# ml-unito/PartitionedLS.jl

Hardware: NVIDIA B200
Metric: opt_fit_orthant_nnls_solves_per_sec (higher is better)
Workload: dtype f64

## Files before the change

### partitionedls.jl_b200/csrc/nnls5.cu

```cuda
#include "common.cuh"

namespace pls {
namespace {

constexpr int H5_BYTES_ = 192;
constexpr int SG_FREE5 = 2;
constexpr unsigned char ST_INO = 1;
constexpr unsigned char ST_PAS = 2;
constexpr unsigned char ST_BLK = 4;
constexpr unsigned char ST_FAST = 8;
#define SYNC5() __syncthreads()

__device__ __forceinline__ void dmma5(double &d0, double &d1, double a, double b) {
  asm("mma.sync.aligned.m8n8k4.row.col.f64.f64.f64.f64 {%0,%1}, {%2}, {%3}, {%0,%1};\n"
      : "+d"(d0), "+d"(d1) : "d"(a), "d"(b));
}
__device__ __forceinline__ double rcp5(double x) {
  double r;
  asm("rcp.approx.ftz.f64 %0, %1;" : "=d"(r) : "d"(x));
  double e = fma(-x, r, 1.0);
  r = fma(r, e, r);
  e = fma(-x, r, 1.0);
  return fma(r, e, r);
}
__device__ __forceinline__ double wmax5(double v) {
#pragma unroll
  for (int o = 16; o; o >>= 1) v = fmax(v, __shfl_xor_sync(0xffffffffu, v, o));
  return v;
}
__host__ __device__ constexpr int t2_doubles(int nr) { return ((nr / 8) * (nr / 8 + 1) / 2) * 64; }
__device__ __forceinline__ int t2_idx(int i, int j) {
  const int ti = i >> 3, tj = j >> 3;
  return ((((ti * (ti + 1)) >> 1) + tj) << 6) + ((i & 7) << 3) + (j & 7);
}
__device__ __forceinline__ double t2_get(const double *T2, int i, int j) { return i >= j ? T2[t2_idx(i, j)] : T2[t2_idx(j, i)]; }
__device__ __forceinline__ void t2_set(double *T2, int i, int j, double v) {
  const int a = i > j ? i : j, b = i > j ? j : i;
  const int x = t2_idx(a, b);
  T2[x] = v;
  if ((a >> 3) == (b >> 3)) T2[x - ((a & 7) << 3) - (b & 7) + ((b & 7) << 3) + (a & 7)] = v;
}
__device__ __forceinline__ int pan5(int row, int col) { return (row << 3) + (col ^ ((row & 2) << 1)); }

struct Sh5 {
  double *T2;
  double *v;
  double *Pp, *Wp;
  double *yv;
  double *D;
  double *gd;
  double *red;
  int4 *binfo;
  int *ctl;
  short *slot;
  short *rvar;
  short *lst;
  short *lstE;
  short *lstB;
  unsigned short *tmap;
  signed char *sg;
  unsigned char *st;
  unsigned char *grp;
  unsigned char *mk;
};
enum { C_NS = 0, C_OK, C_CNT, C_N, C_NJ, C_NP, C_NLV, C_FLAG };

__host__ __device__ inline size_t sh5_bytes(int NR, int ld1) {
  const int ntl = (NR / 8) * (NR / 8 + 1) / 2;
  return H5_BYTES_ + sizeof(double) * ((size_t)t2_doubles(NR) + ld1 + 16 * (size_t)NR + NR + 64 + 8 + 32 + 16) + sizeof(int) * 16 +
         sizeof(short) * (2 * (size_t)ld1 + 2 * (size_t)NR + 8 + ((ntl + 3) & ~3)) + 3 * (size_t)ld1 + NR + 16 + 16;
}

__device__ __forceinline__ Sh5 make_sh5(int NR, int ld1) {
  extern __shared__ __align__(16) unsigned char smem_raw5[];
  const int ntl = (NR / 8) * (NR / 8 + 1) / 2;
  Sh5 s;
  double *dp = reinterpret_cast<double *>(smem_raw5 + H5_BYTES_);
  s.T2 = dp; dp += t2_doubles(NR);
  s.Pp = dp; dp += 8 * NR;
  s.Wp = dp; dp += 8 * NR;
  s.yv = dp; dp += NR;
  s.D = dp; dp += 64;
  s.gd = dp; dp += 8;
  s.red = dp; dp += 32;
  s.binfo = reinterpret_cast<int4 *>(dp); dp += 16;
  int *ip = reinterpret_cast<int *>(dp);
  s.ctl = ip; ip += 16;
  short *sp = reinterpret_cast<short *>(ip);
  s.rvar = sp; sp += NR;
  s.lstE = sp; sp += NR;
  s.lstB = sp; sp += 8;
  s.tmap = reinterpret_cast<unsigned short *>(sp); sp += (ntl + 3) & ~3;
  s.mk = reinterpret_cast<unsigned char *>(sp);
  dp = reinterpret_cast<double *>(smem_raw5 + ((static_cast<int>(s.mk - smem_raw5) + NR + 15) & ~15));
  s.v = dp; dp += ld1;
  sp = reinterpret_cast<short *>(dp);
  s.slot = sp; sp += ld1;
  s.lst = sp; sp += ld1;
  signed char *cp = reinterpret_cast<signed char *>(sp);
  s.sg = cp; cp += ld1;
  s.st = reinterpret_cast<unsigned char *>(cp); cp += ld1;
  s.grp = reinterpret_cast<unsigned char *>(cp);
  return s;
}

struct H5 {
  double *T1;
  const double *T1r;
  double *Pg;
  const double *G;
  const unsigned long long *gmask;
  int ld1, nr, Mp, ldg;
  int cold_fused;
  int gen;
  int pad0, pad1;
  unsigned long long cnt[10];
  double yy, cmax;
  double max_viol;
};
enum { H_SWEEP = 0, H_STREAM, H_SUMS, H_SUMP2, H_ITER, H_BLK, H_REBUILD, H_FOLD, H_DRIFT, H_NOCONV };
constexpr int H5_BYTES = H5_BYTES_;
static_assert(sizeof(H5) <= H5_BYTES, "header size");
__device__ __forceinline__ H5 &hdr5() {
  extern __shared__ __align__(16) unsigned char smem_raw5[];
  return *reinterpret_cast<H5 *>(smem_raw5);
}

template <int T>
__device__ __forceinline__ double bmax5(const Sh5 &s, double v) {
  constexpr int NW = T / 32;
  v = wmax5(v);
  if ((threadIdx.x & 31) == 0) s.red[threadIdx.x >> 5] = v;
  SYNC5();
  double r = s.red[0];
#pragma unroll
  for (int i = 1; i < NW; ++i) r = fmax(r, s.red[i]);
  SYNC5();
  return r;
}

template <int T>
__device__ __forceinline__ void set_block5(const Sh5 &s, int nb, int slot) {
  const int tid = threadIdx.x;
  const H5 &h = hdr5();
  const int g = h.gen;
  if (g == 1) {
    #pragma unroll 1
    for (int k = tid; k < h.nr; k += T) s.mk[k] = 0;
    SYNC5();
  }
  if (tid < nb) {
    const int tc = slot >> 3, c7 = slot & 7;
    s.lstB[tid] = (short)slot;
    s.binfo[tid] = make_int4(slot, (tc << 6) + c7, (((tc * (tc + 1)) >> 1) << 6) + (c7 << 3), 0);
    s.mk[slot] = (unsigned char)g;
  }
}

template <int T, int NR>
__device__ __noinline__ int t2_block(int n, int nb, int nlv, bool test, bool flip) {
  H5 &h = hdr5();
  const int gen = h.gen;
  const Sh5 s = make_sh5(NR, h.ld1);
  constexpr int NW = T / 32;
  const int tid = threadIdx.x, lane = tid & 31, wid = tid >> 5;
  const int fr = lane >> 2, fk = lane & 3;
  const int ntr = (n + 7) >> 3;
  const short *B = s.lstB;
  if (tid >= 32 || T == 32) {
    constexpr int TG = T == 32 ? 32 : T - 32;
#pragma unroll 1
    for (int row = T == 32 ? tid : tid - 32; row < ntr * 8; row += TG) {
      const int tr = row >> 3, r7 = row & 7;
      const int rbase = (((tr * (tr + 1)) >> 1) << 6) + (r7 << 3), rowt = (tr << 6) + r7;
      const int sw = (row & 2) << 1, pb = row << 3;
#pragma unroll 1
      for (int q = 0; q < 8; ++q) {
        double val = 0.0;
        if (row < n && q < nb) { const int4 bi = s.binfo[q]; val = s.T2[row >= bi.x ? rbase + bi.y : bi.z + rowt]; }
        s.Pp[pb + (q ^ sw)] = val;
      }
    }
  }
  if (tid < 32) {
    if (lane < 8) {
      s.gd[lane] = (test && lane >= nlv && lane < nb) ? 1e-13 * __ldg(h.G + (size_t)h.ldg * s.rvar[B[lane]] + s.rvar[B[lane]]) : 0.0;
    }
    const int i = lane >> 2, j0 = (lane & 3) << 1;
    double e0 = (i < nb && j0 < nb) ? t2_get(s.T2, B[i], B[j0]) : (i == j0 ? 1.0 : 0.0);
    double e1 = (i < nb && j0 + 1 < nb) ? t2_get(s.T2, B[i], B[j0 + 1]) : (i == j0 + 1 ? 1.0 : 0.0);
    int bad = nb;
#pragma unroll 1
    for (int k = 0; k < nb; ++k) {
      __syncwarp();
      s.D[i * 8 + j0] = e0; s.D[i * 8 + j0 + 1] = e1;
      __syncwarp();
      const double pk0 = s.D[k * 8 + j0], pk1 = s.D[k * 8 + j0 + 1], cik = s.D[i * 8 + k], pkk = s.D[k * 8 + k];
      const bool good = k < nlv ? pkk < 0.0 : (test ? pkk > s.gd[k] : pkk > 0.0);
      if (!good && bad == nb) bad = k;
      const double d = rcp5(pkk), fct = cik * d;
      const bool rowk = i == k;
      double n0 = rowk ? pk0 * d : fma(-fct, pk0, e0);
      double n1 = rowk ? pk1 * d : fma(-fct, pk1, e1);
      if (j0 == k) n0 = rowk ? d : -fct;
      if (j0 + 1 == k) n1 = rowk ? d : -fct;
      e0 = n0; e1 = n1;
    }
    __syncwarp();
    s.D[i * 8 + j0] = e0; s.D[i * 8 + j0 + 1] = e1;
    if (lane == 0) s.ctl[C_OK] = bad == nb ? nb : (bad < nlv ? -1 : bad);
  }
  SYNC5();
  const int res = s.ctl[C_OK];
  if (tid == 0) h.gen = gen == 255 ? 1 : gen + 1;
  if (res != nb) { SYNC5(); return res; }
  #pragma unroll 1
  for (int ti = wid; ti < ntr; ti += NW) {
    double c0 = 0.0, c1 = 0.0;
// ... 23 lines not shown
    }
  }
  SYNC5();
#pragma unroll 1
  for (int row = tid; row < n; row += T) {
    if (s.mk[row] == (unsigned char)gen) continue;
    const int tr = row >> 3, r7 = row & 7;
    const int rbase = (((tr * (tr + 1)) >> 1) << 6) + (r7 << 3), rowt = (tr << 6) + r7;
    const int sw = (row & 2) << 1, pb = row << 3;
#pragma unroll 1
    for (int q = 0; q < nb; ++q) {
      const int4 bi = s.binfo[q];
      const int tc = bi.x >> 3;
      const double w0 = s.Wp[pb + (q ^ sw)];
      const double val = q < nlv ? -w0 : w0;
      if (tr >= tc) s.T2[rbase + bi.y] = val;
      if (tr <= tc) s.T2[bi.z + rowt] = val;
    }
  }
#pragma unroll 1
  for (int e = tid; e < 64; e += T) {
    const int i = e >> 3, j = e & 7;
    if (i < nb && j <= i) { const double val = s.D[i * 8 + j]; t2_set(s.T2, B[i], B[j], ((i < nlv) == (j < nlv)) ? -val : val); }
  }
  if (flip && tid < nb) s.st[s.rvar[B[tid]]] ^= ST_PAS;
  SYNC5();
  if (tid == 0) { h.cnt[H_SWEEP] += nb; h.cnt[H_SUMP2] += ((unsigned long long)(n * n) * nb) >> 2; }
  return nb;
}

template <int T, int NR>
__device__ __noinline__ bool t2_rebuild(int n) {
  const H5 &h = hdr5();
  const Sh5 s = make_sh5(NR, h.ld1);
  constexpr int NW = T / 32;
  const int tid = threadIdx.x, lane = tid & 31, wid = tid >> 5;
  #pragma unroll 1
  for (int i = wid; i < n; i += NW) {
    const double *row = h.T1r + (size_t)h.ld1 * s.rvar[i];
    #pragma unroll 1
    for (int j = lane; j <= i; j += 32) t2_set(s.T2, i, j, __ldcg(row + s.rvar[j]));
  }
  if (tid < 32) {
    int cnt = 0, nlv = 0;
    #pragma unroll 1
    for (int pass = 0; pass < 2; ++pass) {
      #pragma unroll 1
      for (int k0 = 1; k0 < n; k0 += 32) {
        const int k = k0 + lane;
        bool take = false;
        if (k < n) { const unsigned char f = s.st[s.rvar[k]]; const bool pas = f & ST_PAS, ino = f & ST_INO; take = pas != ino && (pass == 0 ? !pas : pas); }
        const unsigned bal = __ballot_sync(0xffffffffu, take);
        if (take) s.lst[cnt + __popc(bal & ((1u << lane) - 1))] = (short)k;
        cnt += __popc(bal);
      }
      if (pass == 0) nlv = cnt;
    }
    if (lane == 0) { s.ctl[C_CNT] = cnt; s.ctl[C_NLV] = nlv; }
  }
  SYNC5();
  const int cnt = s.ctl[C_CNT], nlv = s.ctl[C_NLV];
  #pragma unroll 1
  for (int q0 = 0; q0 < cnt; q0 += 8) {
    const int nb = min(8, cnt - q0);
    set_block5<T>(s, nb, tid < nb ? s.lst[q0 + tid] : 0);
    SYNC5();
    if (t2_block<T, NR>(n, nb, max(0, min(nb, nlv - q0)), false, false) != nb) return false;
  }
  return true;
}

template <int NR>
__device__ __noinline__ int window_reset() {
  const H5 &h = hdr5();
  const Sh5 s = make_sh5(NR, h.ld1);
  const int tid = threadIdx.x;
  const int Mp = h.Mp;
  if (tid < 32) {
    const int lane = tid;
    if (lane == 0) s.rvar[0] = (short)Mp;
    int base = 1;
    #pragma unroll 1
    for (int m0 = 0; m0 < Mp; m0 += 32) {
      const int m = m0 + lane;
      bool keep = false;
      if (m < Mp) {
        const unsigned char f = s.st[m];
        keep = (f & ST_FAST) || (((f & ST_PAS) != 0) != ((f & ST_INO) != 0));
      }
      const unsigned bal = __ballot_sync(0xffffffffu, keep);
      if (m < Mp) {
        if (keep) { const int k = base + __popc(bal & ((1u << lane) - 1)); s.rvar[k] = (short)m; s.slot[m] = (short)k; }
        else s.slot[m] = -1;
      }
      base += __popc(bal);
    }
    if (lane == 0) s.ctl[C_N] = base;
  }
  SYNC5();
  return s.ctl[C_N];
}

template <int T, int NR>
__device__ __noinline__ int t2_compact(int n) {
  const H5 &h = hdr5();
  const Sh5 s = make_sh5(NR, h.ld1);
  const int tid = threadIdx.x;
  double *scr = h.Pg + 8 * (size_t)h.ld1;
  short *old = s.lst;
  if (tid < 32) {
    const int lane = tid;
    if (lane == 0) old[0] = 0;
    int base = 1;
    #pragma unroll 1
    for (int k0 = 1; k0 < n; k0 += 32) {
      const int k = k0 + lane;
      bool keep = false; int m = 0;
      if (k < n) {
        m = s.rvar[k];
        const unsigned char f = s.st[m];
        keep = (f & ST_FAST) || (((f & ST_PAS) != 0) != ((f & ST_INO) != 0));
      }
      const unsigned bal = __ballot_sync(0xffffffffu, keep);
      const int kn = base + __popc(bal & ((1u << lane) - 1));
      __syncwarp();
      if (k < n) {
        if (keep) { old[kn] = (short)k; s.rvar[kn] = (short)m; s.slot[m] = (short)kn; }
        else s.slot[m] = -1;
      }
      __syncwarp();
      base += __popc(bal);
    }
    if (lane == 0) s.ctl[C_N] = base;
  }
  SYNC5();
  const int nn = s.ctl[C_N];
  if (nn == n) return n;
  #pragma unroll 1
  for (int idx = tid; idx < nn * nn; idx += T) {
    const int a = idx / nn, b = idx - a * nn;
    if (b <= a) __stcg(scr + idx, t2_get(s.T2, old[a], old[b]));
  }
  __threadfence_block();
  SYNC5();
  #pragma unroll 1
  for (int idx = tid; idx < nn * nn; idx += T) {
    const int a = idx / nn, b = idx - a * nn;
    if (b <= a) t2_set(s.T2, a, b, __ldcg(scr + idx));
  }
  SYNC5();
  return nn;
}

template <int T, int NQ, int NR>
__device__ __noinline__ void stream5(int n) {
  const H5 &h = hdr5();
  const Sh5 s = make_sh5(NR, h.ld1);
  const int tid = threadIdx.x;
  const int ld2 = h.ld1 >> 1;
  constexpr int UB = 8;
  constexpr int NG = T >= 512 ? 2 : 1, TG = T / NG, NQE = NQ * NG, UBG = UB * NG;
  const int grp = NG == 1 ? 0 : tid / TG, lt = NG == 1 ? tid : tid - grp * TG;
  int ns = 0;
  {
    constexpr int NW = T / 32;
    const int lane = tid & 31, wid = tid >> 5;
    int *ri = reinterpret_cast<int *>(s.red);
    #pragma unroll 1
    for (int k0 = 1; k0 < n; k0 += T) {
      const int k = k0 + tid;
      bool tg = false, pas = false; int m = 0;
      if (k < n) { m = s.rvar[k]; const unsigned char f = s.st[m]; pas = f & ST_PAS; tg = pas != ((f & ST_INO) != 0); }
      const unsigned bal = __ballot_sync(0xffffffffu, tg);
      if (k0 > 1) SYNC5();
      if (lane == 0) ri[wid] = __popc(bal);
      SYNC5();
      int off = ns;
#pragma unroll
      for (int w2 = 0; w2 < NW; ++w2) { const int c = ri[w2]; if (w2 < wid) off += c; ns += c; }
      if (tg) { const int p = off + __popc(bal & ((1u << lane) - 1)); s.lst[p] = (short)m; const double t = s.T2[t2_idx(k, 0)]; s.yv[p] = pas ? t : -t; }
    }
    const int nsp = (ns + UBG - 1) / UBG * UBG;
    #pragma unroll 1
    for (int p = ns + tid; p < nsp; p += T) { s.lst[p] = (short)h.Mp; s.yv[p] = 0.0; }
    if (tid == 0) { s.ctl[C_NS] = ns; s.ctl[C_FLAG] = 0; }
  }
  SYNC5();
  const int nsp = (ns + UBG - 1) / UBG * UBG;
  double2 acc[NQE];
  const double2 *T1v = reinterpret_cast<const double2 *>(h.T1r);
  {
    const double2 *r = T1v + (size_t)ld2 * h.Mp;
#pragma unroll
    for (int q = 0; q < NQE; ++q) acc[q] = (grp == 0 && lt + TG * q < ld2) ? __ldcg(r + lt + TG * q) : make_double2(0.0, 0.0);
  }
  #pragma unroll 1
  for (int p = 0; p < nsp; p += UBG) {
    double2 g[UB][NQE];
#pragma unroll
    for (int u = 0; u < UB; ++u) {
      const double2 *r = T1v + (size_t)ld2 * s.lst[p + u * NG + grp];
#pragma unroll
      for (int q = 0; q < NQE; ++q) g[u][q] = (lt + TG * q < ld2) ? __ldcg(r + lt + TG * q) : make_double2(0.0, 0.0);
    }
#pragma unroll
    for (int u = 0; u < UB; ++u) {
      const double y = s.yv[p + u * NG + grp];
#pragma unroll
      for (int q = 0; q < NQE; ++q) { acc[q].x = fma(-y, g[u][q].x, acc[q].x); acc[q].y = fma(-y, g[u][q].y, acc[q].y); }
    }
  }
  if (NG > 1) {
    double2 *scr = reinterpret_cast<double2 *>(s.Wp);
    if (grp == 1) {
#pragma unroll
      for (int q = 0; q < NQE; ++q) if (lt + TG * q < ld2) scr[lt + TG * q] = acc[q];
    }
    SYNC5();
    if (grp == 0) {
#pragma unroll
      for (int q = 0; q < NQE; ++q) if (lt + TG * q < ld2) { const double2 o = scr[lt + TG * q]; acc[q].x += o.x; acc[q].y += o.y; }
    }
  }
  if (grp == 0) {
#pragma unroll
    for (int q = 0; q < NQE; ++q)
      if (lt + TG * q < ld2) reinterpret_cast<double2 *>(s.v)[lt + TG * q] = acc[q];
  }
  SYNC5();
  if (tid == 0) { hdr5().cnt[H_STREAM]++; hdr5().cnt[H_SUMS] += ns; }
}

template <int T, int NR>
__device__ __noinline__ int join_block5(int n, const short *Jl, int nj) {
  const H5 &h = hdr5();
  const Sh5 s = make_sh5(NR, h.ld1);
  constexpr int NW = T / 32, TPW = (NR / 8 + NW - 1) / NW;
  const int tid = threadIdx.x, lane = tid & 31, wid = tid >> 5;
  const int fr = lane >> 2, fk = lane & 3;
  const size_t ld1 = h.ld1;
  const double *T1r = h.T1r;
  int nk = 0, m_r = -1, m_c0 = -1, m_c1 = -1, m_t = -1;
  #pragma unroll 1
  for (int q = 0; q < nj; ++q) {
    const int m = Jl[q];
    if (s.slot[m] >= 0) continue;
    if (nk == tid) m_t = m;
    if (nk == fr) m_r = m;
    if (nk == 2 * fk) m_c0 = m;
    if (nk == 2 * fk + 1) m_c1 = m;
    ++nk;
  }
  const auto untoggled = [&](int j) {
    if (j <= 0 || j >= n) return j == 0;
    const unsigned char f = s.st[s.rvar[j]];
    return ((f & ST_PAS) != 0) == ((f & ST_INO) != 0);
  };
  double2 acc[TPW];
#pragma unroll
  for (int u = 0; u < TPW; ++u) {
    const int j = (wid + u * NW) * 8 + fr;
    double x0 = 0.0, x1 = 0.0;
    if (untoggled(j)) {
      const int vj = s.rvar[j];
      if (m_c0 >= 0) x0 = __ldcg(T1r + ld1 * m_c0 + vj);
      if (m_c1 >= 0) x1 = __ldcg(T1r + ld1 * m_c1 + vj);
    }
    acc[u] = make_double2(x0, x1);
  }
  double2 blk = make_double2(0.0, 0.0);
  if (wid == NW - 1 && m_r >= 0) {
    if (m_c0 >= 0) blk.x = __ldcg(T1r + ld1 * m_r + m_c0);
    if (m_c1 >= 0) blk.y = __ldcg(T1r + ld1 * m_r + m_c1);
  }
  int ns = 0;
  {
    int *ri = reinterpret_cast<int *>(s.red);
    #pragma unroll 1
    for (int k0 = 1; k0 < n; k0 += T) {
      const int k = k0 + tid;
      const bool tg = k < n && !untoggled(k);
      const unsigned bal = __ballot_sync(0xffffffffu, tg);
      if (k0 > 1) SYNC5();
      if (lane == 0) ri[wid] = __popc(bal);
      SYNC5();
      int off = ns;
#pragma unroll
      for (int w2 = 0; w2 < NW; ++w2) { const int c = ri[w2]; if (w2 < wid) off += c; ns += c; }
      if (tg) {
        const int p = off + __popc(bal & ((1u << lane) - 1)), var = s.rvar[k];
        const double e = (s.st[var] & ST_PAS) ? 1.0 : -1.0;
        s.lstE[p] = (short)k;
        int a = 0;
        #pragma unroll 1
        for (int q = 0; q < nj; ++q) {
          const int m = Jl[q];
          if (s.slot[m] < 0) s.Pp[pan5(p, a++)] = e * __ldcg(T1r + ld1 * m + var);
        }
        #pragma unroll 1
        for (; a < 8; ++a) s.Pp[pan5(p, a)] = 0.0;
      }
    }
  }
  SYNC5();
  {
    const int ntr = (n + 7) >> 3;
    double2 acc2[TPW];
#pragma unroll
    for (int u = 0; u < TPW; ++u) acc2[u] = make_double2(0.0, 0.0);
    #pragma unroll 1
    for (int k0 = 0; k0 < ns; k0 += 8) {
      const int p0 = k0 + fk, p1 = k0 + 4 + fk;
      const int s0 = p0 < ns ? s.lstE[p0] : 0, s1 = p1 < ns ? s.lstE[p1] : 0;
      const double b0 = p0 < ns ? -s.Pp[pan5(p0, fr)] : 0.0, b1 = p1 < ns ? -s.Pp[pan5(p1, fr)] : 0.0;
#pragma unroll
      for (int u = 0; u < TPW; ++u) {
        const int j = (wid + u * NW) * 8 + fr;
        if (wid + u * NW < ntr) {
          dmma5(acc[u].x, acc[u].y, t2_get(s.T2, j, s0), b0);
          dmma5(acc2[u].x, acc2[u].y, t2_get(s.T2, j, s1), b1);
        }
      }
    }
#pragma unroll
    for (int u = 0; u < TPW; ++u)
      if (wid + u * NW < ntr) {
        const int j = (wid + u * NW) * 8 + fr;
        *reinterpret_cast<double2 *>(s.Wp + pan5(j, 2 * fk)) = make_double2(acc[u].x + acc2[u].x, acc[u].y + acc2[u].y);
      }
  }
  SYNC5();
  if (wid == NW - 1) {
    double2 blk2 = make_double2(0.0, 0.0);
    #pragma unroll 1
    for (int k0 = 0; k0 < ns; k0 += 8) {
      const int p0 = k0 + fk, p1 = k0 + 4 + fk;
      const double a0 = p0 < ns ? -s.Pp[pan5(p0, fr)] : 0.0, a1 = p1 < ns ? -s.Pp[pan5(p1, fr)] : 0.0;
      const double b0 = p0 < ns ? s.Wp[pan5(s.lstE[p0], fr)] : 0.0, b1 = p1 < ns ? s.Wp[pan5(s.lstE[p1], fr)] : 0.0;
      dmma5(blk.x, blk.y, a0, b0);
      dmma5(blk2.x, blk2.y, a1, b1);
    }
    if (fr < nk && 2 * fk <= fr) t2_set(s.T2, n + fr, n + 2 * fk, blk.x + blk2.x);
    if (fr < nk && 2 * fk + 1 <= fr) t2_set(s.T2, n + fr, n + 2 * fk + 1, blk.y + blk2.y);
  }
  if (tid < nk) { s.rvar[n + tid] = (short)m_t; s.slot[m_t] = (short)(n + tid); }
  #pragma unroll 1
  for (int idx = tid; idx < nk * n; idx += T) {
    const int a = idx / n, j = idx - a * n;
    t2_set(s.T2, n + a, j, s.Wp[pan5(j, a)]);
  }
  if (tid == 0) hdr5().cnt[H_SUMP2] += ((unsigned long long)ns * n * nk) >> 1;
  SYNC5();
  return nk;
}

template <int T, int NR>
__device__ __noinline__ bool fold_block5(int boff, int nb) {
  H5 &h = hdr5();
  const Sh5 s = make_sh5(NR, h.ld1);
  const short *B = s.lstE + boff;
  constexpr int NW = T / 32;
  const int tid = threadIdx.x, lane = tid & 31, wid = tid >> 5;
  const int fr = lane >> 2, fk = lane & 3;
  const int ld1 = h.ld1, nt = ld1 >> 3;
  double *FP = s.T2, *FW = s.T2 + (size_t)ld1 * 8;
  #pragma unroll 1
  for (int idx = tid; idx < ld1 * 8; idx += T) {
    const int j = idx >> 3, q = idx & 7;
    FP[pan5(j, q)] = q < nb ? __ldcg(h.T1r + (size_t)ld1 * B[q] + j) : 0.0;
  }
  if (tid < 8) s.gd[tid] = (tid < nb && (s.st[B[tid]] & ST_PAS)) ? 1e-13 * __ldg(h.G + (size_t)h.ldg * B[tid] + B[tid]) : 0.0;
  SYNC5();
  if (tid < 32) {
    bool ok = true;
    const int i = lane >> 2, j0 = (lane & 3) << 1;
    double e0 = (i < nb && j0 < nb) ? FP[pan5(B[i], j0)] : (i == j0 ? 1.0 : 0.0);
    double e1 = (i < nb && j0 + 1 < nb) ? FP[pan5(B[i], j0 + 1)] : (i == j0 + 1 ? 1.0 : 0.0);
    #pragma unroll 1
    for (int k = 0; k < nb; ++k) {
      __syncwarp();
// ... 160 lines not shown
    int tj = q - ((ti * (ti + 1)) >> 1);
    #pragma unroll 1
    for (; q < q1; ++q) {
      double2 c = __ldcg(reinterpret_cast<const double2 *>(h.T1r + (size_t)(ti * 8 + fr) * ld1 + tj * 8 + 2 * fk));
      const double *za = ZT + (size_t)(ti * 8 + fr) * nk + fk, *pb = rows + tj * 8 + fr;
#pragma unroll 1
      for (int t0 = 0; t0 < ntr; t0 += CH) {
        double z0[CH], z1[CH], p0[CH], p1[CH];
#pragma unroll
        for (int u = 0; u < CH; ++u) {
          const bool live = t0 + u < ntr;
          const int k = (t0 + u) * 8 + fk;
          z0[u] = live ? za[(t0 + u) * 8] : 0.0; z1[u] = live ? za[(t0 + u) * 8 + 4] : 0.0;
          p0[u] = live ? __ldcg(pb + roff[k]) : 0.0; p1[u] = live ? __ldcg(pb + roff[k + 4]) : 0.0;
        }
#pragma unroll
        for (int u = 0; u < CH; ++u) { dmma5(c.x, c.y, z0[u], p0[u]); dmma5(c.x, c.y, z1[u], p1[u]); }
      }
      __stcg(reinterpret_cast<double2 *>(h.T1 + (size_t)(ti * 8 + fr) * ld1 + tj * 8 + 2 * fk), c);
      if (ti != tj) {
        double *mp = h.T1 + (size_t)(tj * 8 + 2 * fk) * ld1 + ti * 8 + fr;
        __stcg(mp, c.x); __stcg(mp + ld1, c.y);
      }
      if (++tj > ti) { ++ti; tj = 0; }
    }
  }
  SYNC5();
  #pragma unroll 1
  for (int k = 1; k < n; ++k) {
    const double e = s.yv[k];
    if (e == 0.0) continue;
    const int var = s.rvar[k];
    #pragma unroll 1
    for (int j = tid; j < ld1; j += T) {
      const double val = -e * ZT[(size_t)j * nk + k];
      __stcg(h.T1 + (size_t)ld1 * var + j, val);
      __stcg(h.T1 + (size_t)ld1 * j + var, val);
    }
  }
  SYNC5();
  #pragma unroll 1
  for (int idx = tid; idx < n * n; idx += T) {
    const int a = idx / n, b = idx - a * n;
    __stcg(h.T1 + (size_t)ld1 * s.rvar[a] + s.rvar[b], t2_get(s.T2, a, b));
  }
  SYNC5();
  #pragma unroll 1
  for (int k = tid; k < n; k += T) {
    if (k >= 1 && s.yv[k] != 0.0) { const int m = s.rvar[k]; const unsigned char f = s.st[m]; s.st[m] = (f & ST_PAS) ? (unsigned char)(f | ST_INO) : (unsigned char)(f & ~ST_INO); }
  }
  if (tid == 0) { h.T1r = h.T1; h.cnt[H_SUMP2] += 2ull * ld1 * ld1 * (unsigned long long)ntr / 8 + (unsigned long long)ld1 * nk * nk / 2; h.cnt[H_FOLD]++; }
  SYNC5();
}

template <int T, int NR>
__device__ __noinline__ int fold5(int n, bool cold_mode) {
  const H5 &h = hdr5();
  const Sh5 s = make_sh5(NR, h.ld1);
  const int tid = threadIdx.x;
  if (cold_mode) n = t2_compact<T, NR>(n);
  short *B = s.lstE;
  if (tid < 32) {
    const int lane = tid;
    int cnt = 0;
    #pragma unroll 1
    for (int pass = 0; pass < 2; ++pass) {
      #pragma unroll 1
      for (int k0 = 1; k0 < n; k0 += 32) {
        const int k = k0 + lane;
        bool take = false; int m = 0;
        if (k < n) {
          m = s.rvar[k];
          const unsigned char f = s.st[m];
          const bool pas = f & ST_PAS, ino = f & ST_INO;
          take = pas != ino && !(f & ST_FAST) && (pass == 0 ? !pas : pas);
        }
        const unsigned bal = __ballot_sync(0xffffffffu, take);
        if (take) B[cnt + __popc(bal & ((1u << lane) - 1))] = (short)m;
        cnt += __popc(bal);
      }
    }
    if (lane == 0) s.ctl[C_CNT] = cnt;
  }
  SYNC5();
  const int cnt = s.ctl[C_CNT];
  bool ok = true;
  if (cold_mode && cnt > 8 && h.cold_fused) fold_fused5<T, NR>(n);
  else for (int q0 = 0; q0 < cnt && ok; q0 += 8) ok = fold_block5<T, NR>(q0, min(8, cnt - q0));
  n = window_reset<NR>();
  if (!t2_rebuild<T, NR>(n)) ok = false;
  return ok ? n : -1;
}

template <int T, int NR>
__device__ __noinline__ double verify5(const double *c) {
  const H5 &h = hdr5();
  const Sh5 s = make_sh5(NR, h.ld1);
  const int tid = threadIdx.x;
  const int Mp = h.Mp;
  double *wf = h.Pg;
  if (tid < 32) {
    const int lane = tid;
    int np = 0;
    #pragma unroll 1
    for (int m0 = 0; m0 < Mp; m0 += 32) {
      const int m = m0 + lane;
      bool pas = false; double wv = 0.0;
      if (m < Mp) {
        pas = s.st[m] & ST_PAS;
        if (pas) wv = s.slot[m] >= 0 ? s.T2[t2_idx(s.slot[m], 0)] : s.v[m];
      }
      const unsigned bal = __ballot_sync(0xffffffffu, pas);
      if (pas) { const int p = np + __popc(bal & ((1u << lane) - 1)); s.lst[p] = (short)m; wf[p] = wv; }
      np += __popc(bal);
    }
    if (lane == 0) s.ctl[C_NP] = np;
  }
  SYNC5();
  const int np = s.ctl[C_NP];
  double mx = 0.0;
  #pragma unroll 1
  for (int m = tid; m < Mp; m += T) {
    double a0 = c[m], a1 = 0.0;
    int t = 0;
    #pragma unroll 1
    for (; t + 1 < np; t += 2) {
      a0 = fma(-h.G[(size_t)h.ldg * s.lst[t] + m], wf[t], a0);
      a1 = fma(-h.G[(size_t)h.ldg * s.lst[t + 1] + m], wf[t + 1], a1);
    }
    if (t < np) a0 = fma(-h.G[(size_t)h.ldg * s.lst[t] + m], wf[t], a0);
    const double rv = a0 + a1;
    const int sg = s.sg[m];
    const unsigned char f = s.st[m];
    if (f & ST_PAS) mx = fmax(mx, fabs(rv));
    else if (sg == SG_FREE5) mx = fmax(mx, fabs(rv));
    else if (sg != 0 && !(f & ST_BLK)) mx = fmax(mx, (double)sg * rv);
  }
  return bmax5<T>(s, mx);
}

template <int T, int NR, int NQ>
__device__ __forceinline__ bool solve5(const Sh5 s, int &n_win, bool cold_mode, bool &t2_fresh) {
  const int tid = threadIdx.x;
  H5 &h = hdr5();
  const int Mp = h.Mp;
  const double cmax = h.cmax;
  const double told = 1e-12 * cmax;
  int t_best = Mp + 1, pbar = 3, iters = 0, rebuilt = 0;
  #pragma unroll 1
  for (;;) {
    #pragma unroll 1
    for (;;) {
      const int n = n_win;
      int nl = 0, ne = 0, mx = -1;
      {
        constexpr int NW = T / 32;
        const int lane = tid & 31, wid = tid >> 5;
        int4 *ri = reinterpret_cast<int4 *>(s.red);
        #pragma unroll 1
        for (int k0 = 1; k0 < n; k0 += T) {
          const int k = k0 + tid;
          int f = 0, m = -1;
          if (k < n) {
            m = s.rvar[k];
            const double val = s.T2[t2_idx(k, 0)];
            const int sg = s.sg[m];
            const unsigned char fl = s.st[m];
            if (fl & ST_PAS) { if (sg != SG_FREE5 && (sg == 0 || (double)sg * val < 0.0)) f = 1; }
            else if (!(fl & ST_BLK) && sg != 0 && (sg == SG_FREE5 ? fabs(val) > told : (double)sg * val > told)) f = 2;
          }
          const unsigned bl = __ballot_sync(0xffffffffu, f == 1), be = __ballot_sync(0xffffffffu, f == 2);
          const int mw = __reduce_max_sync(0xffffffffu, f ? m : -1);
          if (k0 > 1) SYNC5();
          if (lane == 0) ri[wid] = make_int4(__popc(bl), __popc(be), mw, 0);
          SYNC5();
          int ol = nl, oe = ne;
#pragma unroll
          for (int w2 = 0; w2 < NW; ++w2) {
            const int4 r = ri[w2];
            if (w2 < wid) { ol += r.x; oe += r.y; }
            nl += r.x; ne += r.y; mx = max(mx, r.z);
          }
          const unsigned below = (1u << lane) - 1;
          if (f == 1) s.lst[ol + __popc(bl & below)] = (short)k;
          if (f == 2) s.lstE[oe + __popc(be & below)] = (short)k;
        }
      }
      SYNC5();
      const int nv = nl + ne;
      if (nv == 0) break;
      if (tid == 0) h.cnt[H_ITER]++;
      if (++iters > 60 + 6 * Mp) return false;
      bool single = false;
      if (nv < t_best) { t_best = nv; pbar = 3; }
      else if (pbar >= 1) --pbar;
      else single = true;
      if (single) {
        const int k = s.slot[mx];
        const bool pas = s.st[mx] & ST_PAS;
        nl = pas ? 1 : 0; ne = pas ? 0 : 1;
        SYNC5();
        if (tid == 0) { if (pas) s.lst[0] = (short)k; else s.lstE[0] = (short)k; }
        SYNC5();
      }
      t2_fresh = false;
      int done = 0, tot = nl + ne;
      bool broken = false;
      while (done < tot) {
        const int nb = min(8, tot - done), nlv = max(0, min(nb, nl - done));
        set_block5<T>(s, nb, tid < nb ? (done + tid < nl ? s.lst[done + tid] : s.lstE[done + tid - nl]) : 0);
        SYNC5();
        const int r = t2_block<T, NR>(n, nb, nlv, true, true);
        if (r == nb) { done += nb; continue; }
        if (r < 0) { broken = true; break; }
        const int pos = done + r - nl;
        if (tid == 0) {
          s.st[s.rvar[s.lstE[pos]]] |= ST_BLK;
          #pragma unroll 1
          for (int q = pos; q + 1 < ne; ++q) s.lstE[q] = s.lstE[q + 1];
        }
        --ne; --tot; if (tid == 0) h.cnt[H_BLK]++;
        SYNC5();
      }
      if (broken) {
        if (++rebuilt > 3 || !t2_rebuild<T, NR>(n)) return false;
        t2_fresh = true; if (tid == 0) h.cnt[H_REBUILD]++;
      }
    }
    stream5<T, NQ, NR>(n_win);
    {
      const int ns = s.ctl[C_NS];
      int code = 0;
#pragma unroll 1
      for (int p = tid; p < ns; p += T) if (!(fabs(s.v[s.lst[p]]) <= 1e-12 * cmax)) code |= 2;
#pragma unroll 1
      for (int m = tid; m < Mp; m += T) {
        if (s.slot[m] < 0) {
          const int sg = s.sg[m];
          const unsigned char fl = s.st[m];
          const double val = s.v[m];
          bool f;
          if (fl & ST_INO) f = sg != SG_FREE5 && (sg == 0 ? val != 0.0 : (double)sg * val < 0.0);
          else f = !(fl & ST_BLK) && sg != 0 && (sg == SG_FREE5 ? fabs(val) > told : (double)sg * val > told);
          if (f) code |= 1;
        }
      }
      if (code) atomicOr(&s.ctl[C_FLAG], code);
      SYNC5();
      const int flags = s.ctl[C_FLAG];
      if (flags & 2) {
        double res = 0.0;
#pragma unroll 1
        for (int p = tid; p < ns; p += T) { const double r = fabs(s.v[s.lst[p]]); res = r == r ? fmax(res, r) : r; }
        res = bmax5<T>(s, res);
        if (res != res || (t2_fresh && res > 1e-9 * cmax) || ++rebuilt > 3) return false;
        if (!t2_rebuild<T, NR>(n_win)) return false;
        t2_fresh = true;
        if (tid == 0) h.cnt[H_REBUILD]++;
        continue;
      }
      if (!(flags & 1)) return true;
    }
    if (tid < 32) {
      const int lane = tid;
      int nj = 0;
#pragma unroll 1
      for (int m0 = 0; m0 < Mp; m0 += 32) {
        const int m = m0 + lane;
        bool f = false;
        if (m < Mp && s.slot[m] < 0) {
          const int sg = s.sg[m];
          const unsigned char fl = s.st[m];
          const double val = s.v[m];
          if (fl & ST_INO) f = sg != SG_FREE5 && (sg == 0 ? val != 0.0 : (double)sg * val < 0.0);
          else f = !(fl & ST_BLK) && sg != 0 && (sg == SG_FREE5 ? fabs(val) > told : (double)sg * val > told);
        }
        const unsigned bal = __ballot_sync(0xffffffffu, f);
        if (f) s.lst[nj + __popc(bal & ((1u << lane) - 1))] = (short)m;
        nj += __popc(bal);
      }
      if (lane == 0) s.ctl[C_NJ] = nj;
    }
    SYNC5();
    const int nj = s.ctl[C_NJ];
    if (nj == 0) return true;
    if (++iters > 60 + 6 * Mp) return false;
    if (NR - n_win < nj) {
      short *park = reinterpret_cast<short *>(s.v);
      #pragma unroll 1
      for (int p = tid; p < nj; p += T) park[p] = s.lst[p];
      SYNC5();
      if (cold_mode) n_win = t2_compact<T, NR>(n_win);
      if (NR - n_win < (nj < 8 ? nj : 8)) {
        const int nf = fold5<T, NR>(n_win, cold_mode);
        if (nf < 0) return false;
        n_win = nf;
        t2_fresh = true;
      }
      int room = NR - n_win;
      if (room > nj) room = nj;
      if (room <= 0) return false;
      #pragma unroll 1
      for (int p = 0; p < room; p += 8) n_win += join_block5<T, NR>(n_win, park + p, min(8, room - p));
    } else {
      #pragma unroll 1
      for (int p = 0; p < nj; p += 8) n_win += join_block5<T, NR>(n_win, s.lst + p, min(8, nj - p));
    }
    t_best = Mp + 1; pbar = 3;
  }
}

template <int T, int NR>
__device__ __noinline__ void cold_init5(const double *T0) {
  H5 &h = hdr5();
  const Sh5 s = make_sh5(NR, h.ld1);
  const int tid = threadIdx.x, ld1 = h.ld1;
  if (tid == 0) h.T1r = T0;
  #pragma unroll 1
  for (int m = tid; m < ld1; m += T) { s.st[m] = 0; s.slot[m] = -1; s.sg[m] = 0; }
  SYNC5();
}

__global__ void __launch_bounds__(128) k2v5_build_t0(const double *G, int ldg, const double *c, const double *scal, int Mp, int ld1, double *T0) {
  const int row = blockIdx.x;
  for (int col = threadIdx.x; col < ld1; col += blockDim.x) {
    double val = 0.0;
    if (row < Mp) val = col < Mp ? G[(size_t)ldg * row + col] : (col == Mp ? c[row] : 0.0);
    else if (row == Mp) val = col < Mp ? c[col] : (col == Mp ? scal[0] : 0.0);
    T0[(size_t)ld1 * row + col] = val;
  }
}

template <int T>
__device__ __forceinline__ void set_lowmask5(const Sh5 &s, unsigned long long mask) {
  const H5 &h = hdr5();
  #pragma unroll 1
  for (int m = threadIdx.x; m < h.Mp; m += T) {
    const unsigned char f = s.st[m];
    s.st[m] = (h.gmask[m] & mask) ? (unsigned char)(f | ST_FAST) : (unsigned char)(f & ~ST_FAST);
  }
  SYNC5();
}

template <int T>
__device__ __forceinline__ void set_signs5(const Sh5 &s, long long b, int free_top, int Kp, int fb) {
  const H5 &h = hdr5();
  #pragma unroll 1
  for (int m = threadIdx.x; m < h.Mp; m += T) {
    const int g = s.grp[m];
    if (fb >= 0 && g != 255) {
      if (g == fb) s.sg[m] = (signed char)-s.sg[m];
    } else if (fb < 0 || ((h.gmask[m] >> fb) & 1ull)) {
      const unsigned long long gm = h.gmask[m];
      const int d = 2 * __popcll(gm & (unsigned long long)b) - __popcll(gm);
      const bool fr = free_top && ((gm >> (Kp - 1)) & 1ull);
      s.sg[m] = (signed char)(fr ? SG_FREE5 : (d > 0) - (d < 0));
    }
    s.st[m] &= (unsigned char)~ST_BLK;
  }
  SYNC5();
}

template <int T, int NR, int NQ, int MINB>
__global__ void __launch_bounds__(T, MINB) k2v5_orthant_walks(const K2Args A) {
  const int tid = threadIdx.x;
  const int Mp = A.Mp, ld1 = A.cap;
  const Sh5 s = make_sh5(NR, ld1);
  H5 &h = hdr5();
  if (tid == 0) {
    h.T1 = A.tab + (size_t)blockIdx.x * A.tabstride; h.ld1 = ld1; h.T1r = A.hglob;
    h.Pg = h.T1 + (size_t)ld1 * ld1;
    h.Mp = Mp; h.nr = NR; h.cold_fused = A.chain_log2; h.gen = 1;
    h.gmask = reinterpret_cast<const unsigned long long *>(A.gmask);
    h.G = A.G; h.ldg = A.ldg;
    #pragma unroll 1
    for (int q = 0; q < 10; ++q) h.cnt[q] = 0;
    h.yy = A.scal[0]; h.cmax = A.scal[1]; h.max_viol = 0.0;
  }
  int n_win = 1;
  bool cold_mode = true;
  #pragma unroll 1
  for (int ti = tid; ti < NR / 8; ti += T)
    #pragma unroll 1
    for (int tj = 0; tj <= ti; ++tj) s.tmap[((ti * (ti + 1)) >> 1) + tj] = (unsigned short)((ti << 8) | tj);
  #pragma unroll 1
  for (int k = tid; k < NR; k += T) s.mk[k] = 0;
  #pragma unroll 1
  for (int m = tid; m < Mp; m += T) { const unsigned long long gm = reinterpret_cast<const unsigned long long *>(A.gmask)[m]; s.grp[m] = (unsigned char)(__popcll(gm) == 1 ? __ffsll((long long)gm) - 1 : 255); }
  #pragma unroll 1
  for (int e = tid; e < t2_doubles(NR); e += T) s.T2[e] = 0.0;
  double best_obj = 0.0; long long best_b = -1;
  int low_bits = 0;
  while ((A.lowmask >> low_bits) & 1ull) ++low_bits;
  const long long cnt = A.n_chains;
  const long long i0 = cnt * (long long)blockIdx.x / (long long)gridDim.x;
  const long long i1 = cnt * ((long long)blockIdx.x + 1) / (long long)gridDim.x;
  bool cold = true, just_cold = false, t2_fresh = true;
  int since_check = 0, check_every = A.verify_every;
  SYNC5();

  #pragma unroll 1
  for (long long i = i0; i < i1; ++i) {
    if (cold) {
      cold_init5<T, NR>(A.hglob);
      cold_mode = true;
      n_win = window_reset<NR>();
      t2_rebuild<T, NR>(n_win);
      cold = false; just_cold = true; since_check = 0; t2_fresh = true;
    }
    const long long b = A.b_begin + (i ^ (i >> 1));
    const int fb = i > 0 ? __ffsll(i) - 1 : 63;
    set_signs5<T>(s, b, A.free_top, A.Kp, (just_cold || i == i0) ? -1 : fb);

    const bool ok = solve5<T, NR, NQ>(s, n_win, cold_mode, t2_fresh);
    if (!ok) { cold = true; if (tid == 0) h.cnt[H_NOCONV]++; }

    ++since_check;
    if (ok && (since_check >= check_every || i + 1 == i1)) {
      since_check = 0;
      const double viol = verify5<T, NR>(A.c);
      const double cmax = h.cmax;
      if (!just_cold && tid == 0) h.max_viol = fmax(h.max_viol, viol);
      if (viol > 1e-13 * cmax && check_every > 8) check_every = 8;
      if (viol > 1e-12 * cmax && !just_cold) { if (tid == 0) h.cnt[H_DRIFT]++; cold = true; --i; continue; }
    }
    just_cold = false;

    const double obj = ok ? sqrt(fmax(s.v[Mp], 0.0)) : __longlong_as_double(0x7ff8000000000000ll);
    const long long rel = b - A.b_begin;
    double w_top = 0.0;
    if (A.free_top && (s.st[Mp - 1] & ST_PAS)) w_top = s.slot[Mp - 1] >= 0 ? s.T2[t2_idx(s.slot[Mp - 1], 0)] : s.v[Mp - 1];
    const long long b_full = A.free_top ? (b | ((w_top > 0.0 ? 1ll : 0ll) << (A.Kp - 1))) : b;
    if (A.all_obj && tid == 0) A.all_obj[rel] = obj;
    const bool better = opt_better(obj, b_full, best_obj, best_b, PLS_TIE_REL * h.yy);
    if (better) { best_obj = obj; best_b = b_full; }
    if (A.all_alpha || better) {
      #pragma unroll 1
      for (int m = tid; m < Mp; m += T) {
        const unsigned long long gm = h.gmask[m];
        const int d = 2 * __popcll(gm & (unsigned long long)b) - __popcll(gm);
        double wv = 0.0;
        if (ok && (s.st[m] & ST_PAS)) wv = s.slot[m] >= 0 ? s.T2[t2_idx(s.slot[m], 0)] : s.v[m];
        const double al = s.sg[m] == SG_FREE5 ? fabs(wv) : (d != 0 ? fmax(wv / (double)d, 0.0) : 0.0);
        if (A.all_alpha) A.all_alpha[(size_t)rel * Mp + m] = al;
        if (better) A.cta_w[(size_t)blockIdx.x * Mp + m] = al;
      }
    }
    if (ok) {
      bool tslow = false;
#pragma unroll 1
      for (int k = tid + 1; k < n_win; k += T) {
        const int m = s.rvar[k]; const unsigned char f = s.st[m];
        tslow = tslow || ((((f & ST_PAS) != 0) != ((f & ST_INO) != 0)) && !(f & ST_FAST));
      }
      const int nslow = __syncthreads_count(tslow);
      const bool was_cold = cold_mode;
      if (fb >= low_bits || nslow >= 8 || n_win > NR - 8 || was_cold) {
        const int nf = fold5<T, NR>(n_win, cold_mode);
        if (nf < 0) cold = true;
        else n_win = nf;
        t2_fresh = true;
        if (was_cold && !cold) {
          set_lowmask5<T>(s, A.lowmask);
          cold_mode = false;
          n_win = window_reset<NR>();
          if (!t2_rebuild<T, NR>(n_win)) cold = true;
        }
      }
    }
    SYNC5();
  }
  if (tid == 0) {
    A.cta_obj[blockIdx.x] = best_obj;
    A.cta_b[blockIdx.x] = best_b;
    atomicAdd(&A.counters[CNT_PIVOTS], h.cnt[H_SWEEP]);
    atomicAdd(&A.counters[CNT_GRAD], h.cnt[H_STREAM]);
    atomicAdd(&A.counters[CNT_SUMP], h.cnt[H_SUMS]);
    atomicAdd(&A.counters[CNT_SUMP2], h.cnt[H_SUMP2]);
    atomicAdd(&A.counters[CNT_ITERS], h.cnt[H_ITER]);
    atomicAdd(&A.counters[CNT_REBUILDS], h.cnt[H_REBUILD]);
    atomicAdd(&A.counters[CNT_BLOCKED], h.cnt[H_BLK]);
    atomicAdd(&A.counters[CNT_NOCONV], h.cnt[H_NOCONV]);
    atomicAdd(&A.counters[CNT_SPILLS], h.cnt[H_DRIFT]);
    atomicMax(&A.counters[CNT_DRIFT], (unsigned long long)__double_as_longlong(h.max_viol / h.cmax));
    atomicAdd(&A.counters[CNT_V5_FOLDS], h.cnt[H_FOLD]);
  }
}

typedef void (*K5Fn)(const K2Args);
struct Variant5 { int T, NR, NQ, minb; K5Fn fn; };
#define V5(T, NR, NQ, MINB) {T, NR, NQ, MINB, k2v5_orthant_walks<T, NR, NQ, MINB>}
const Variant5 kVariants5[] = {
    V5(128, 64, 1, 7), V5(128, 72, 1, 6), V5(128, 80, 1, 5), V5(128, 96, 1, 4), V5(64, 64, 2, 7), V5(64, 72, 2, 6), V5(64, 80, 2, 5), V5(64, 96, 2, 4),
    V5(32, 72, 4, 6),
    V5(128, 96, 2, 4),
    V5(512, 160, 1, 1), V5(512, 192, 1, 1), V5(512, 208, 1, 1),
};
#undef V5

}

int k2v5_plan(int Mp, int n_bits, const uint64_t *h_gmask, K5Plan *pl) {
  if (!h_gmask) return PLS_EUNSUPPORTED;
  const int ld1 = (Mp + 1 + 7) & ~7;
  const char *eT = getenv("PLS_K5_T"), *eN = getenv("PLS_K5_NR");
  const int wantT = eT ? atoi(eT) : 0, wantNR = eN ? atoi(eN) : 0;
  int dev = 0, max_smem = 0;
  PLS_CUDA_TRY(cudaGetDevice(&dev));
  PLS_CUDA_TRY(cudaDeviceGetAttribute(&max_smem, cudaDevAttrMaxSharedMemoryPerBlockOptin, dev));
  const Variant5 *v = nullptr;
  int vi = -1, l = 0;
  const char *eM = getenv("PLS_K5_MARGIN");
  const int margin = eM ? atoi(eM) : 12;
  const int l_want = n_bits - 2 < 6 ? (n_bits - 2 < 1 ? 1 : n_bits - 2) : 6;
  int ci = 0;
  for (const Variant5 &c : kVariants5) {
    const bool fits = c.T == (wantT ? wantT : (ld1 > 328 ? 512 : 128)) && (!wantNR || c.NR == wantNR) && ld1 <= 2 * c.T * c.NQ &&
                      2 * (size_t)ld1 * 8 <= (size_t)t2_doubles(c.NR) + 16 * (size_t)c.NR && sh5_bytes(c.NR, ld1) <= (size_t)max_smem;
    if (fits) {
      int lc = 0;
      for (int t = 1; t <= n_bits && t <= 10; ++t) {
        int nf = 0;
        const uint64_t mask = (1ull << t) - 1ull;
        for (int m = 0; m < Mp; ++m) nf += (h_gmask[m] & mask) != 0ull;
        if (nf + 1 + margin <= c.NR) lc = t; else break;
      }
      if (lc > l) { v = &c; vi = ci; l = lc; }
      if (l >= l_want) break;
    }
    ++ci;
  }
  if (!v || l < 1) return PLS_EUNSUPPORTED;
  if (const char *eL = getenv("PLS_K5_L")) { const int t = atoi(eL); if (t >= 1 && t < l) l = t; }
  const size_t sm = sh5_bytes(v->NR, ld1);
  PLS_CUDA_TRY(cudaFuncSetAttribute(v->fn, cudaFuncAttributeMaxDynamicSharedMemorySize, (int)sm));
  int oc = 1;
  PLS_CUDA_TRY(cudaOccupancyMaxActiveBlocksPerMultiprocessor(&oc, v->fn, v->T, sm));
  if (oc < 1) oc = 1;
  if (const char *eO = getenv("PLS_K5_OCC")) { const int o = atoi(eO); if (o >= 1 && o < oc) oc = o; }
  pl->variant = vi; pl->T = v->T; pl->NR = v->NR; pl->ld1 = ld1; pl->occ = oc; pl->smem = sm; pl->low_groups = l;
  pl->tabstride = (size_t)ld1 * ld1 + 8 * (size_t)ld1 + 2 * (size_t)ld1 * v->NR + 64;
  const char *eV = getenv("PLS_K5_VERIFY");
  pl->verify_every = eV ? atoi(eV) : 128;
  const char *eF = getenv("PLS_K5_FUSED");
  pl->cold_fused = v->NR > 96 ? 0 : (eF ? atoi(eF) : 1);
  if (pl->verify_every < 1) pl->verify_every = 1;
  return PLS_OK;
}

int k2v5_launch(const K2Args &A, const K5Plan &pl, int grid, cudaStream_t st) {
  k2v5_build_t0<<<pl.ld1, 128, 0, st>>>(A.G, A.ldg, A.c, A.scal, A.Mp, pl.ld1, A.hglob);
  PLS_CUDA_TRY(cudaGetLastError());
  kVariants5[pl.variant].fn<<<grid, pl.T, pl.smem, st>>>(A);
  PLS_CUDA_TRY(cudaGetLastError());
  return PLS_OK;
}

}
```

Before: 36.56 million.

## Fuse violation scan, stream list build and slow-count into fewer block passes

When the window fits in one thread pass (NR <= T), the violation scan in solve5 now also builds the stream list and counts slow variables, so stream5 skips its own scan and barrier. The post-stream KKT check is folded into stream5's write-back of v, and the separate tslow reduction after a solve is replaced by a count kept in shared memory. Together these remove several block-wide barriers and shared-memory passes per active-set iteration. The price is more duplicated, fragile logic. The fused residual check now tests slot/state flags instead of the list, and the stored slow count may be stale relative to the final state.

```diff
diff --git a/partitionedls.jl_b200/csrc/nnls5.cu b/partitionedls.jl_b200/csrc/nnls5.cu
--- a/partitionedls.jl_b200/csrc/nnls5.cu
+++ b/partitionedls.jl_b200/csrc/nnls5.cu
@@ -63,7 +63,7 @@
   unsigned char *grp;
   unsigned char *mk;
 };
-enum { C_NS = 0, C_OK, C_CNT, C_N, C_NJ, C_NP, C_NLV, C_FLAG };
+enum { C_NS = 0, C_OK, C_CNT, C_N, C_NJ, C_NP, C_NLV, C_FLAG, C_NSLOW };
 
 __host__ __device__ inline size_t sh5_bytes(int NR, int ld1) {
   const int ntl = (NR / 8) * (NR / 8 + 1) / 2;
@@ -393,6 +393,8 @@
   return nn;
 }
 
+template <int T> constexpr int NG5 = T >= 512 ? 2 : 1;
+template <int T> constexpr int UBG5 = 8 * NG5<T>;
 template <int T, int NQ, int NR>
 __device__ __noinline__ void stream5(int n) {
   const H5 &h = hdr5();
@@ -400,10 +402,12 @@
   const int tid = threadIdx.x;
   const int ld2 = h.ld1 >> 1;
   constexpr int UB = 8;
-  constexpr int NG = T >= 512 ? 2 : 1, TG = T / NG, NQE = NQ * NG, UBG = UB * NG;
+  constexpr int NG = NG5<T>, TG = T / NG, NQE = NQ * NG, UBG = UBG5<T>;
   const int grp = NG == 1 ? 0 : tid / TG, lt = NG == 1 ? tid : tid - grp * TG;
   int ns = 0;
-  {
+  if constexpr (NR <= T) {
+    ns = s.ctl[C_NS];
+  } else {
     constexpr int NW = T / 32;
     const int lane = tid & 31, wid = tid >> 5;
     int *ri = reinterpret_cast<int *>(s.red);
@@ -425,8 +429,8 @@
     #pragma unroll 1
     for (int p = ns + tid; p < nsp; p += T) { s.lst[p] = (short)h.Mp; s.yv[p] = 0.0; }
     if (tid == 0) { s.ctl[C_NS] = ns; s.ctl[C_FLAG] = 0; }
-  }
-  SYNC5();
+    SYNC5();
+  }
   const int nsp = (ns + UBG - 1) / UBG * UBG;
   double2 acc[NQE];
   const double2 *T1v = reinterpret_cast<const double2 *>(h.T1r);
@@ -464,9 +468,31 @@
     }
   }
   if (grp == 0) {
+    const int Mp = h.Mp;
+    const double told = 1e-12 * h.cmax;
+    int code = 0;
+    const auto check = [&](int m, double val) {
+      if (m >= Mp) return;
+      const int sg = s.sg[m];
+      const unsigned char fl = s.st[m];
+      if (s.slot[m] >= 0) {
+        if (((fl & ST_PAS) != 0) != ((fl & ST_INO) != 0) && !(fabs(val) <= told)) code |= 2;
+      } else {
+        bool f;
+        if (fl & ST_INO) f = sg != SG_FREE5 && (sg == 0 ? val != 0.0 : (double)sg * val < 0.0);
+        else f = !(fl & ST_BLK) && sg != 0 && (sg == SG_FREE5 ? fabs(val) > told : (double)sg * val > told);
+        if (f) code |= 1;
+      }
+    };
 #pragma unroll
     for (int q = 0; q < NQE; ++q)
-      if (lt + TG * q < ld2) reinterpret_cast<double2 *>(s.v)[lt + TG * q] = acc[q];
+      if (lt + TG * q < ld2) {
+        const int j = lt + TG * q;
+        reinterpret_cast<double2 *>(s.v)[j] = acc[q];
+        check(2 * j, acc[q].x);
+        check(2 * j + 1, acc[q].y);
+      }
+    if (code) atomicOr(&s.ctl[C_FLAG], code);
   }
   SYNC5();
   if (tid == 0) { hdr5().cnt[H_STREAM]++; hdr5().cnt[H_SUMS] += ns; }
@@ -933,8 +959,50 @@
     #pragma unroll 1
     for (;;) {
       const int n = n_win;
-      int nl = 0, ne = 0, mx = -1;
-      {
+      int nl = 0, ne = 0, mx = -1, nslow = 0;
+      if constexpr (NR <= T) {
+        constexpr int NW = T / 32;
+        const int lane = tid & 31, wid = tid >> 5;
+        int4 *ri = reinterpret_cast<int4 *>(s.red);
+        const int k = 1 + tid;
+        int f = 0, m = -1;
+        bool tg = false, pas = false, slow = false;
+        double val = 0.0;
+        if (k < n) {
+          m = s.rvar[k];
+          val = s.T2[t2_idx(k, 0)];
+          const int sg = s.sg[m];
+          const unsigned char fl = s.st[m];
+          pas = fl & ST_PAS;
+          tg = pas != ((fl & ST_INO) != 0);
+          slow = tg && !(fl & ST_FAST);
+          if (pas) { if (sg != SG_FREE5 && (sg == 0 || (double)sg * val < 0.0)) f = 1; }
+          else if (!(fl & ST_BLK) && sg != 0 && (sg == SG_FREE5 ? fabs(val) > told : (double)sg * val > told)) f = 2;
+        }
+        const unsigned bl = __ballot_sync(0xffffffffu, f == 1), be = __ballot_sync(0xffffffffu, f == 2);
+        const unsigned bt = __ballot_sync(0xffffffffu, tg), bs = __ballot_sync(0xffffffffu, slow);
+        const int mw = __reduce_max_sync(0xffffffffu, f ? m : -1);
+        if (lane == 0) ri[wid] = make_int4(__popc(bl), __popc(be), mw, __popc(bt) | (__popc(bs) << 16));
+        SYNC5();
+        int ol = 0, oe = 0, os = 0, ns = 0;
+#pragma unroll
+        for (int w2 = 0; w2 < NW; ++w2) {
+          const int4 r = ri[w2];
+          if (w2 < wid) { ol += r.x; oe += r.y; os += r.w & 0xffff; }
+          nl += r.x; ne += r.y; mx = max(mx, r.z); ns += r.w & 0xffff; nslow += r.w >> 16;
+        }
+        const unsigned below = (1u << lane) - 1;
+        if (nl + ne == 0) {
+          if (tg) { const int p = os + __popc(bt & below); s.lst[p] = (short)m; s.yv[p] = pas ? val : -val; }
+          const int nsp = (ns + UBG5<T> - 1) / UBG5<T> * UBG5<T>;
+          #pragma unroll 1
+          for (int p = ns + tid; p < nsp; p += T) { s.lst[p] = (short)Mp; s.yv[p] = 0.0; }
+          if (tid == 0) { s.ctl[C_NS] = ns; s.ctl[C_FLAG] = 0; }
+        } else {
+          if (f == 1) s.lst[ol + __popc(bl & below)] = (short)k;
+          if (f == 2) s.lstE[oe + __popc(be & below)] = (short)k;
+        }
+      } else {
         constexpr int NW = T / 32;
         const int lane = tid & 31, wid = tid >> 5;
         int4 *ri = reinterpret_cast<int4 *>(s.red);
@@ -942,31 +1010,35 @@
         for (int k0 = 1; k0 < n; k0 += T) {
           const int k = k0 + tid;
           int f = 0, m = -1;
+          bool slow = false;
           if (k < n) {
             m = s.rvar[k];
             const double val = s.T2[t2_idx(k, 0)];
             const int sg = s.sg[m];
             const unsigned char fl = s.st[m];
+            slow = (((fl & ST_PAS) != 0) != ((fl & ST_INO) != 0)) && !(fl & ST_FAST);
             if (fl & ST_PAS) { if (sg != SG_FREE5 && (sg == 0 || (double)sg * val < 0.0)) f = 1; }
             else if (!(fl & ST_BLK) && sg != 0 && (sg == SG_FREE5 ? fabs(val) > told : (double)sg * val > told)) f = 2;
           }
           const unsigned bl = __ballot_sync(0xffffffffu, f == 1), be = __ballot_sync(0xffffffffu, f == 2);
+          const unsigned bs = __ballot_sync(0xffffffffu, slow);
           const int mw = __reduce_max_sync(0xffffffffu, f ? m : -1);
           if (k0 > 1) SYNC5();
-          if (lane == 0) ri[wid] = make_int4(__popc(bl), __popc(be), mw, 0);
+          if (lane == 0) ri[wid] = make_int4(__popc(bl), __popc(be), mw, __popc(bs) << 16);
           SYNC5();
           int ol = nl, oe = ne;
 #pragma unroll
           for (int w2 = 0; w2 < NW; ++w2) {
             const int4 r = ri[w2];
             if (w2 < wid) { ol += r.x; oe += r.y; }
-            nl += r.x; ne += r.y; mx = max(mx, r.z);
+            nl += r.x; ne += r.y; mx = max(mx, r.z); nslow += r.w >> 16;
           }
           const unsigned below = (1u << lane) - 1;
           if (f == 1) s.lst[ol + __popc(bl & below)] = (short)k;
           if (f == 2) s.lstE[oe + __popc(be & below)] = (short)k;
         }
       }
+      if (tid == 0) s.ctl[C_NSLOW] = nslow;
       SYNC5();
       const int nv = nl + ne;
       if (nv == 0) break;
@@ -1011,23 +1083,6 @@
     stream5<T, NQ, NR>(n_win);
     {
       const int ns = s.ctl[C_NS];
-      int code = 0;
-#pragma unroll 1
-      for (int p = tid; p < ns; p += T) if (!(fabs(s.v[s.lst[p]]) <= 1e-12 * cmax)) code |= 2;
-#pragma unroll 1
-      for (int m = tid; m < Mp; m += T) {
-        if (s.slot[m] < 0) {
-          const int sg = s.sg[m];
-          const unsigned char fl = s.st[m];
-          const double val = s.v[m];
-          bool f;
-          if (fl & ST_INO) f = sg != SG_FREE5 && (sg == 0 ? val != 0.0 : (double)sg * val < 0.0);
-          else f = !(fl & ST_BLK) && sg != 0 && (sg == SG_FREE5 ? fabs(val) > told : (double)sg * val > told);
-          if (f) code |= 1;
-        }
-      }
-      if (code) atomicOr(&s.ctl[C_FLAG], code);
-      SYNC5();
       const int flags = s.ctl[C_FLAG];
       if (flags & 2) {
         double res = 0.0;
@@ -1228,15 +1283,9 @@
       }
     }
     if (ok) {
-      bool tslow = false;
-#pragma unroll 1
-      for (int k = tid + 1; k < n_win; k += T) {
-        const int m = s.rvar[k]; const unsigned char f = s.st[m];
-        tslow = tslow || ((((f & ST_PAS) != 0) != ((f & ST_INO) != 0)) && !(f & ST_FAST));
-      }
-      const int nslow = __syncthreads_count(tslow);
       const bool was_cold = cold_mode;
-      if (fb >= low_bits || nslow >= 8 || n_win > NR - 8 || was_cold) {
+      if (fb >= low_bits || s.ctl[C_NSLOW] >= 8 || n_win > NR - 8 || was_cold) {
+        SYNC5();
         const int nf = fold5<T, NR>(n_win, cold_mode);
         if (nf < 0) cold = true;
         else n_win = nf;
```

Measured after the change: 37.59 million (median of 6 runs). 2.8% higher.
